# vpecanins/stm32f7-rtlsdr

Hardware: AMD Instinct MI355X
Metric: IQ MSamples/s through FIR+FM-demod+resample (higher is better)
Workload: dtype f32 audio; K2 = u8 x 24-bit fixed-point taps on the i8 matrix pipe, exact i32 sums, one f32 recombination (design Q); K3 / K4 f32; ill-conditioned phases recomputed with the f32 fmaf chain

## Files before the change

### stm32f7-rtlsdr_amd/csrc/sdrfm_q.hip

```cpp
#include <hip/hip_runtime.h>
#include <hip/hip_ext.h>

#include <cstddef>
#include <cstdint>
#include <type_traits>

#include "sdrfm_math.h"
#include "sdrfm_q.h"
#include "sdrfm_b.h"

typedef int qi4_t __attribute__((ext_vector_type(4)));
typedef int qi8_t __attribute__((ext_vector_type(8)));
typedef float qf2_t __attribute__((ext_vector_type(2)));
__device__ void q_raw_buffer_load_lds(qi4_t rsrc, __attribute__((address_space(3))) void* lds, int size, int voffset, int soffset,
                                      int offset, int aux) __asm("llvm.amdgcn.raw.buffer.load.lds");

namespace {

constexpr int QTA = (int)SDRFM_Q_TA;
constexpr int DB0 = 128;
constexpr int ABS = 4;
constexpr int ABW = 128 * ABS;
constexpr int FLW = 64 + 2;
#ifndef SDRFM_Q_GTAB
// ... 39 lines not shown
#define SDRFM_Q_WQB 4
#endif
constexpr int WQB = SDRFM_Q_WQB;
static_assert(WQB >= 4 && WQB <= 16 && 8 * WQB >= (int)SDRFM_Q_TA, "a warm-up holds the d history of a run's first audio output");

__device__ __forceinline__ float q_discriminate(float yr, float yi, float pr, float pi) {
  const float re = __builtin_fmaf(yr, pr, yi * pi);
  const float im = yi * pr - yr * pi;
  const float ax = __builtin_fabsf(re), ay = __builtin_fabsf(im);
  const float mx = __builtin_fmaxf(__builtin_fmaxf(ax, ay), 0x1p-120f), mn = __builtin_fminf(ax, ay);
  const float v = mn * __builtin_amdgcn_rcpf(mx);
  const float s2 = v * v;
  float q = 0x1.e34882p-8f;
  q = __builtin_fmaf(q, s2, -0x1.22fc74p-5f);
  q = __builtin_fmaf(q, s2, 0x1.509024p-4f);
  q = __builtin_fmaf(q, s2, -0x1.12688cp-3f);
  q = __builtin_fmaf(q, s2, 0x1.96c562p-3f);
  q = __builtin_fmaf(q, s2, -0x1.554086p-2f);
  float a = __builtin_fmaf(v, s2 * q, v);
  if (ay > ax) a = 0x1.921fb6p+0f - a;
  if (re < 0.0f) a = 0x1.921fb6p+1f - a;
  return __builtin_copysignf(a, im);
}

__device__ __forceinline__ float q_angle(float yr, float yi, float& mx_out) {
  const float ax = __builtin_fabsf(yr), ay = __builtin_fabsf(yi);
  const float mx = __builtin_fmaxf(__builtin_fmaxf(ax, ay), 0x1p-120f), mn = __builtin_fminf(ax, ay);
  mx_out = mx;
  const float v = mn * __builtin_amdgcn_rcpf(mx);
  const float s2 = v * v;
  float q = 0x1.e34882p-8f;
  q = __builtin_fmaf(q, s2, -0x1.22fc74p-5f);
  q = __builtin_fmaf(q, s2, 0x1.509024p-4f);
  q = __builtin_fmaf(q, s2, -0x1.12688cp-3f);
  q = __builtin_fmaf(q, s2, 0x1.96c562p-3f);
  q = __builtin_fmaf(q, s2, -0x1.554086p-2f);
  float a = __builtin_fmaf(v, s2 * q, v);
  if (ay > ax) a = 0x1.921fb6p+0f - a;
  if (yr < 0.0f) a = 0x1.921fb6p+1f - a;
  return __builtin_copysignf(a, yi);
}
__device__ __forceinline__ float q_wrap(float x) {
  float t = __builtin_fmaf(x, 0x1.45f306p-3f, 0x1.8p+23f);
  asm volatile("" : "+v"(t));
  const float k = t - 0x1.8p+23f;
  return __builtin_fmaf(k, -0x1.921fb6p+2f, x);
}

__device__ __forceinline__ unsigned q_pcm_word(float v) {
  const float c = __builtin_amdgcn_fmed3f(v, -32768.0f, 32767.0f);
  float t = c + 0x1.8p+23f;
  asm volatile("" : "+v"(t));
  return __builtin_amdgcn_perm(__builtin_bit_cast(unsigned, t), __builtin_bit_cast(unsigned, t), 0x05040504u);
}

template <int N>
__device__ __forceinline__ void wait_vmcnt() {
  static_assert(N >= 0 && N < 16, "vmcnt immediate");
  __builtin_amdgcn_s_waitcnt(0x0f70 | N);
}

#ifdef SDRFM_Q_PHASES
#define Q_PHASE(i) do { const unsigned long long tn_ = __builtin_readcyclecounter(); t_ph[i] += tn_ - t_last; t_last = tn_; } while (0)
#else
#define Q_PHASE(i) do { } while (0)
#endif

template <int D, int DA, int NSLOT>
constexpr uint32_t q_lds() { return (uint32_t)(QGeo<D, DA>::PRE + 1024 * NSLOT + 4 * (QGeo<D, DA>::DBW + ABW + FLW + GTW)); }
struct QPcmArgs { SdrfmQParams p; SdrfmSinkChain t; };
static_assert(ABS * 128 <= 64 * (int)SDRFM_CHAIN_CH, "a flush of parked audio is one scan of the wave");
template <int C0, int NSLOT, int D, int DA, bool PCM = false>
__device__ __forceinline__ void mfir_body(const SdrfmQParams& p, const uint32_t bid) {
  using G = QGeo<D, DA>;
  [[maybe_unused]] constexpr int NCH = G::NCH;
  constexpr int QD = D, QDA = DA, NSC = G::NSC, BLKB = G::BLKB, STEPB = G::STEPB, PRE = G::PRE, DBW = G::DBW, RWIN = G::RWIN;
  constexpr bool ALIGNED = G::ALIGNED;
  constexpr int CS = G::CS;
  constexpr int RINGB = NSLOT * 1024;
  static_assert(RINGB % (2 * STEPB) == 0 && (ALIGNED ? NSLOT == 2 * CS : (NSLOT >= 5 && NSLOT - 4 < 16)), "ring: whole pairs of steps");
  extern __shared__ __attribute__((aligned(16))) unsigned char smem[];
  float* const db = reinterpret_cast<float*>(smem + PRE + RINGB);
  float* const ab = db + DBW;
  unsigned short* const fl16 = reinterpret_cast<unsigned short*>(ab + ABW);
  const int lane = (int)threadIdx.x, n = lane & 15, g = lane >> 4;
  const uint32_t si = bid / p.runs, run = bid - si * p.runs;
  const uint32_t stream = p.slist ? p.slist[si] : si;
  const uint32_t Bt = (p.M + 7u) >> 3, Qt = (Bt + WQB - 1u) / WQB, vs = p.iq_prev ? 1u : 0u;
  const uint32_t Gq = Qt + p.runs - 1u + vs;
  const uint32_t e0 = (uint32_t)(((uint64_t)run * Gq) / p.runs), e1 = (uint32_t)(((uint64_t)(run + 1) * Gq) / p.runs);
  const int q0 = run == 0 ? 0 : (int)e0 - (int)(run - 1u + vs), q1 = (int)e1 - (int)(run + vs);
  if (q0 >= q1) return;
  if (lane == 0) *reinterpret_cast<uint2*>(fl16 + 128) = make_uint2(0u, 0u);
#ifdef SDRFM_Q_STAMPS
  unsigned long long* const tsp = p.dbg ? p.dbg + 16 * (size_t)bid : nullptr;
  unsigned long long t_wait = 0, t_first = 0;
  const unsigned long long t_entry = __builtin_amdgcn_s_memrealtime();
  const unsigned long long c_entry = __builtin_readcyclecounter();
#endif
#ifdef SDRFM_Q_PHASES
  unsigned long long t_ph[8] = {0, 0, 0, 0, 0, 0, 0, 0}, t_last = 0;
#endif
  const bool from_prev = run == 0 && p.iq_prev != nullptr;
  const bool warm = run > 0 || from_prev;
  const int b0 = WQB * q0;
  int b1 = WQB * q1;
// ... 207 lines not shown
        q_raw_buffer_load_lds(rsrc, slot_ptr(0), 16, vpos, 0, 0, SDRFM_Q_AUX);
        q_raw_buffer_load_lds(rsrc, slot_ptr(0), 16, vpos, 0, 1024, SDRFM_Q_AUX);
        vpos += 2048;
      }
      return;
    }
    if (k > 0 && !(k & 1)) {
      q_raw_buffer_load_lds(rsrc, slot_ptr(slot), 16, vpos, 0, 0, SDRFM_Q_AUX);
      vpos += 1024;
      slot = (slot + 1 == NSLOT) ? 0 : slot + 1;
    }
    q_raw_buffer_load_lds(rsrc, slot_ptr(slot), 16, vpos, 0, 0, SDRFM_Q_AUX);
    q_raw_buffer_load_lds(rsrc, slot_ptr(slot), 16, vpos, 0, 1024, SDRFM_Q_AUX);
    slot = (slot + 2 >= NSLOT) ? slot + 2 - NSLOT : slot + 2;
    vpos += 2048;
  };
  typedef const __attribute__((address_space(4))) SdrfmQParams* KargPtr;
  auto kargs = [&]() -> KargPtr {
    KargPtr pp = (KargPtr)__builtin_amdgcn_kernarg_segment_ptr();
    asm volatile("" : "+s"(pp));
    return pp;
  };
  int npend = 0, jfl = jg0;
  [[maybe_unused]] float yrun = 0.0f;
  [[maybe_unused]] bool pfirst = true;
  [[maybe_unused]] float* const pstash = reinterpret_cast<float*>(smem + q_lds<D, DA, NSLOT>());
  typedef const __attribute__((address_space(4))) SdrfmSinkChain* KChainPtr;
  [[maybe_unused]] auto kchain = [&]() -> KChainPtr {
    const __attribute__((address_space(4))) unsigned char* pp = (const __attribute__((address_space(4))) unsigned char*)__builtin_amdgcn_kernarg_segment_ptr();
    asm volatile("" : "+s"(pp));
    return (KChainPtr)(pp + offsetof(QPcmArgs, t));
  };
  [[maybe_unused]] unsigned long long pv_early = 0ull;
  [[maybe_unused]] bool published = false;
  [[maybe_unused]] float dp_early = 0.0f;
  auto flush_audio = [&](const bool fin = false) {
    __builtin_amdgcn_wave_barrier();
#if defined(SDRFM_Q_ABLATE) && (SDRFM_Q_ABLATE & 256)
    float* row = p.audio - jfl;
    const int ln_ = lane;
#else
    uint32_t st_ = stream;
    int ln_ = lane;
    asm volatile("" : "+s"(st_), "+v"(ln_));
    float* row = kargs()->audio + (size_t)st_ * kargs()->audio_stride;
#endif
    const int lo = jfl > jlo ? jfl : jlo;
#if defined(SDRFM_Q_ABLATE) && (SDRFM_Q_ABLATE & 128)
    const int hi_ = (ab[lane] == 1234.5f) ? lo + 2 : lo;
#else
    const int hi_ = (j1 < jfl + 128 * npend) ? j1 : jfl + 128 * npend;
#endif
    const int par = (int)((reinterpret_cast<uintptr_t>(row) >> 2) & 1u);
    bool want_audio = true;
    if constexpr (PCM) want_audio = kargs()->audio != nullptr;
    if (want_audio) for (int e = lo - ((lo + par) & 1) + 2 * ln_; e < hi_; e += 128) {
      const bool v0 = e >= lo, v1 = e + 1 < hi_;
      const float a0 = v0 ? ab[e - jfl] : 0.0f, a1 = v1 ? ab[e + 1 - jfl] : 0.0f;
      if constexpr (PCM) {
        if (v0 && v1) __builtin_nontemporal_store(qf2_t{a0, a1}, reinterpret_cast<qf2_t*>(row + e));
        else if (v0) __builtin_nontemporal_store(a0, row + e);
        else if (v1) __builtin_nontemporal_store(a1, row + e + 1);
      } else {
        if (v0 && v1) *reinterpret_cast<qf2_t*>(row + e) = qf2_t{a0, a1};
        else if (v0) row[e] = a0;
        else if (v1) row[e + 1] = a1;
      }
    }
    if constexpr (PCM) {
      const int cntf = hi_ - lo;
      if (cntf > 0) {
        constexpr int PCH = (int)SDRFM_CHAIN_CH, FIX = (int)SDRFM_CHAIN_FIX;
        const KChainPtr tp = kchain();
        const float alpha = tp->alpha, gain = tp->gain;
        asm volatile("s_waitcnt lgkmcnt(0)" ::: "memory");
        __builtin_amdgcn_wave_barrier();
        float* const xa = ab + (lo - jfl);
        unsigned* const xw = reinterpret_cast<unsigned*>(xa);
        const int i0 = PCH * ln_;
        float xr[PCH];
#pragma unroll
        for (int q = 0; q < PCH; ++q) xr[q] = (i0 + q < cntf) ? xa[i0 + q] : 0.0f;
        float sc = 0.0f;
#pragma unroll
        for (int q = 0; q < PCH; ++q) sc = __builtin_fmaf(tp->w[q], xr[q], sc);
        float pw = tp->pc;
        if (ln_ == 0) sc = __builtin_fmaf(pw, yrun, sc);
#pragma unroll
        for (int d = 1; d < 64; d <<= 1) {
          const float o = __shfl_up(sc, (unsigned)d, 64);
          const float sn = __builtin_fmaf(pw, o, sc);
          sc = ln_ >= d ? sn : sc;
          pw *= pw;
        }
        if (fin) {
          const int Ll = (cntf - 1) / PCH, rl = (cntf - 1) % PCH;
          const float ypub = __shfl(sc, Ll, 64) * tp->dinv[PCH - 1 - rl];
          uint32_t bid2 = bid;
          asm volatile("" : "+s"(bid2));
          if (ln_ == 0) {
            const uint32_t call = tp->call, nst = tp->n_streams;
            const unsigned long long w = ((unsigned long long)((last_run ? call : tp->run_call) + 1u) << 32) | __builtin_bit_cast(unsigned, ypub);
            __hip_atomic_store(last_run ? tp->sg + (size_t)((call + 1u) % SDRFM_CHAIN_SG_SLOTS) * nst + st_ : tp->runstate + bid2, w, __ATOMIC_RELAXED,
                               __HIP_MEMORY_SCOPE_AGENT);
            unsigned long long zero = 0ull;
            asm volatile("" : "+v"(zero));
            pv_early = __hip_atomic_fetch_add(run == 0 ? tp->sg + (size_t)(call % SDRFM_CHAIN_SG_SLOTS) * nst + st_ : tp->runstate + (bid2 - 1u), zero,
                                              __ATOMIC_RELAXED, __HIP_MEMORY_SCOPE_AGENT);
          }
          dp_early = ln_ < (int)SDRFM_CHAIN_FIX ? tp->dpow[ln_] : 0.0f;
          published = true;
        }
        float y = __shfl_up(sc, 1u, 64);
        if (ln_ == 0) y = yrun;
        __builtin_amdgcn_wave_barrier();
#pragma unroll
        for (int q = 0; q < PCH; ++q) {
          const float yn = __builtin_fmaf(alpha, xr[q] - y, y);
          y = (i0 + q < cntf) ? yn : y;
          if (i0 + q < cntf) {
            xw[i0 + q] = q_pcm_word(yn * gain);
            if (pfirst && i0 + q < FIX) pstash[i0 + q] = yn;
          }
        }
        yrun = __shfl(y, (cntf - 1) / PCH, 64);
        __builtin_amdgcn_wave_barrier();
        unsigned* const out = reinterpret_cast<unsigned*>(tp->pcm + (size_t)st_ * tp->pcm_stride);
        const int parp = (int)((reinterpret_cast<uintptr_t>(out) >> 2) & 1u), ps = lo + (pfirst ? FIX : 0);
        for (int e = ps - ((ps + parp) & 1) + 2 * ln_; e < hi_; e += 128) {
          const bool v0 = e >= ps, v1 = e + 1 < hi_;
          const unsigned w0 = v0 ? xw[e - lo] : 0u, w1 = v1 ? xw[e + 1 - lo] : 0u;
          if (v0 && v1) *reinterpret_cast<uint2*>(out + e) = make_uint2(w0, w1);
          else if (v0) out[e] = w0;
          else if (v1) out[e + 1] = w1;
        }
        pfirst = false;
      }
    }
    jfl += 128 * npend;
    npend = 0;
  };
  int nflag = 0;
  auto repair_flagged = [&]() {
    int ln = lane;
    uint32_t st = stream;
    asm volatile("" : "+v"(ln), "+s"(st));
    const KargPtr pp = kargs();
#ifdef SDRFM_Q_PHASES
    unsigned long long r_t0 = __builtin_readcyclecounter(), r_t1;
#define R_PHASE(word, shift, waitfirst) do { if (waitfirst) asm volatile("s_waitcnt vmcnt(0) lgkmcnt(0)" ::: "memory"); r_t1 = __builtin_readcyclecounter(); \
                                             t_ph[word] += ((r_t1 - r_t0) & 0xffffffffull) << shift; r_t0 = r_t1; } while (0)
#else
#define R_PHASE(word, shift, waitfirst) do { } while (0)
#endif
    const unsigned char* const row = pp->iq + (size_t)st * pp->iq_stride;
    const unsigned char* const pre = from_prev ? pp->iq_prev + (size_t)st * pp->iq_prev_stride + 2 * (size_t)pp->N_prev
                                               : pp->hist_q_in + (size_t)(2 * QTP) * ((size_t)st + 1);
    unsigned* const cnt = reinterpret_cast<unsigned*>(fl16 + 128);
    __builtin_amdgcn_wave_barrier();
    unsigned nrep = 0;
    for (int e0 = 0; e0 < nflag; e0 += 64) {
      const int e = e0 + ln;
      int l = 0, slot = 0, m0 = (int)pp->M;
      if (e < nflag) {
        const unsigned ent = fl16[e];
        l = (int)(ent & 63u);
        slot = (int)(ent >> 6) - 1;
        m0 = mbase + 128 * slot + 8 * (l & 15) + 2 * (l >> 4);
      }
      const bool act = m0 < (int)pp->M;
      nrep += (unsigned)__builtin_popcountll(__builtin_amdgcn_ballot_w64(act));
      if (act) {
        const int n0 = QD * m0 - QTP;
        uint2 w[RWIN / 4];
#pragma unroll
        for (int c = 0; c < RWIN / 4; ++c) {
          const int n = n0 + 4 * c;
          w[c] = *reinterpret_cast<const uint2*>((n >= 0 ? row : pre) + 2 * (ptrdiff_t)n);
        }
        R_PHASE(0, 0, 0);
        R_PHASE(0, 32, 1);
        qf2_t a[3] = {qf2_t{0.0f, 0.0f}, qf2_t{0.0f, 0.0f}, qf2_t{0.0f, 0.0f}};
        const float* const hz = db;
#pragma unroll
        for (int i = 0; i < RWIN; ++i) {
          const unsigned wd = (i & 2) ? w[i >> 2].y : w[i >> 2].x;
          const qf2_t b = {(float)((wd >> ((i & 1) ? 16 : 0)) & 0xffu), (float)((wd >> ((i & 1) ? 24 : 8)) & 0xffu)};
          const qf2_t x = b - qf2_t{127.5f, 127.5f};
// ... 259 lines not shown
      a0 += a0b;
      a1 += a1b;
      *reinterpret_cast<qf2_t*>(ab + 128 * npend + 2 * lane) = qf2_t{a0, a1};
      ++npend;
      if (osm == QDA) {
        if (lane < QTA) {
          const float hv = db[DB0 + sigma + 128 * QDA - QTA + lane];
          db[DB0 + sigma - QTA + lane] = hv;
        }
        __builtin_amdgcn_wave_barrier();
        osm = 0;
        mbase += 128 * QDA;
      }
      if (npend == ABS) flush_audio();
      Q_PHASE(6);
    }
#if SDRFM_Q_PEEL
  };
  for (int kk = 0; kk < nsteps - 1; ++kk) step(std::false_type{}, kk);
  step(std::true_type{}, nsteps - 1);
#else
  }
#endif
#ifdef SDRFM_Q_STAMPS
  const unsigned long long t_loop = __builtin_amdgcn_s_memrealtime();
#endif
  wait_vmcnt<0>();
  flush_audio(true);
  if constexpr (PCM) {
    const KChainPtr tp = kchain();
    uint32_t st_ = stream, bid_ = bid;
    int ln_ = lane;
    asm volatile("" : "+s"(st_), "+s"(bid_), "+v"(ln_));
    const uint32_t call = tp->call, nst = tp->n_streams;
    unsigned long long* const rs = tp->runstate;
    unsigned long long* const sg = tp->sg;
    const float dp = published ? dp_early : (ln_ < (int)SDRFM_CHAIN_FIX ? tp->dpow[ln_] : 0.0f);
    unsigned long long pv = pv_early;
    if (ln_ == 0) {
      if (!published) {
        const unsigned long long w = ((unsigned long long)((last_run ? call : tp->run_call) + 1u) << 32) | __builtin_bit_cast(unsigned, yrun);
        __hip_atomic_store(last_run ? sg + (size_t)((call + 1u) % SDRFM_CHAIN_SG_SLOTS) * nst + st_ : rs + bid_, w, __ATOMIC_RELAXED, __HIP_MEMORY_SCOPE_AGENT);
      }
      unsigned long long* const src = run == 0 ? sg + (size_t)(call % SDRFM_CHAIN_SG_SLOTS) * nst + st_ : rs + (bid_ - 1u);
      const uint32_t want = run == 0 ? call : tp->run_call + 1u;
      unsigned long long zero = 0ull;
      asm volatile("" : "+v"(zero));
      int it = 0;
      for (;; ++it) {
        if (it > 0 || !published) pv = __hip_atomic_fetch_add(src, zero, __ATOMIC_RELAXED, __HIP_MEMORY_SCOPE_AGENT);
        if ((uint32_t)(pv >> 32) == want || it == (1 << 19)) break;
        __builtin_amdgcn_s_sleep(16);
      }
      if (it == (1 << 19)) { pv = 0ull; __hip_atomic_store(tp->err, 1u, __ATOMIC_RELAXED, __HIP_MEMORY_SCOPE_AGENT); }
    }
    const float carry = __builtin_bit_cast(float, __builtin_amdgcn_readfirstlane((int)(unsigned)pv));
    const int nfix = (j1 - jlo < (int)SDRFM_CHAIN_FIX) ? j1 - jlo : (int)SDRFM_CHAIN_FIX;
    if (ln_ < nfix) {
      const float yv = __builtin_fmaf(dp, carry, pstash[ln_]);
      reinterpret_cast<unsigned*>(tp->pcm + (size_t)st_ * tp->pcm_stride)[jlo + ln_] = q_pcm_word(yv * tp->gain);
    }
  }
  const KargPtr pe = kargs();
  if (pe->n_repaired && lane == 0) {
    const uint2 cnt = *reinterpret_cast<const uint2*>(fl16 + 128);
    if (cnt.y) {
      atomicAdd(pe->n_repaired, cnt.x);
      atomicAdd(pe->n_repaired + 1, cnt.y);
      if (pe->stream_pass) atomicAdd(pe->stream_pass + stream, cnt.y);
    }
  }

  if (last_run && !(SDRFM_Q_HO_RING && !ALIGNED)) {
    const unsigned char* row = pe->iq + (size_t)stream * pe->iq_stride;
    const int HTe = (int)pe->T - 1;
    const size_t Ne = pe->N;
    for (int k = lane; k < HTe; k += 64) {
      const unsigned raw = *reinterpret_cast<const unsigned short*>(row + 2 * (Ne - HTe + k));
      reinterpret_cast<unsigned short*>(pe->hist_b_out)[(size_t)stream * HTe + k] = (unsigned short)raw;
      pe->hist_x_out[(size_t)stream * HTe + k] = make_float2((float)(raw & 0xffu) - 127.5f, (float)(raw >> 8) - 127.5f);
    }
    if (lane < 2 * QTP / 16)
      *reinterpret_cast<qi4_t*>(pe->hist_q_out + (size_t)(2 * QTP) * stream + 16 * lane) =
          *reinterpret_cast<const qi4_t*>(row + 2 * Ne - 2 * QTP + 16 * lane);
  }
#ifdef SDRFM_Q_STAMPS
  if (tsp && lane == 0) {
    tsp[0] = t_entry; tsp[1] = t_first; tsp[2] = t_loop; tsp[3] = __builtin_amdgcn_s_memrealtime(); tsp[4] = t_wait;
#ifdef SDRFM_Q_PHASES
    for (int i = 0; i < 8; ++i) tsp[8 + i] = t_ph[i];
#endif
    tsp[5] = (__builtin_amdgcn_s_getreg((3 << 11) | 20) & 7) | ((unsigned long long)__builtin_amdgcn_s_getreg((31 << 11) | 4) << 8);
    tsp[6] = (unsigned long long)nsteps; tsp[7] = __builtin_readcyclecounter() - c_entry;
  }
#endif
}


template <int C0, int NSLOT, int D, int DA>
__global__ void __launch_bounds__(64) __attribute__((amdgpu_waves_per_eu(D == 16 ? 3 : 4))) k_mfir(SdrfmQParams p) {
  mfir_body<C0, NSLOT, D, DA>(p, blockIdx.x);
}

template <int C0, int NSLOT, int D, int DA>
__global__ void __launch_bounds__(64) __attribute__((amdgpu_waves_per_eu(D == 16 ? 3 : 4))) k_mfir_pcm(QPcmArgs a) {
  mfir_body<C0, NSLOT, D, DA, true>(a.p, blockIdx.x);
}
// ... 207 lines not shown
```

### stm32f7-rtlsdr_amd/csrc/sdrfm_sink.hip

```cpp
#include <hip/hip_runtime.h>
#include <hip/hip_ext.h>

#include <cmath>
#include <cstdint>
#include <cstdio>
#include <cstring>
#include <new>

#include "../../include/sdrfm.h"
#include "sdrfm_sink_chain.h"

namespace {

struct SinkParams {
  const float* audio;
  size_t audio_stride;
  int16_t* pcm;
  size_t pcm_stride;
  const unsigned long long* sg_in;
  unsigned long long* sg_out;
  uint32_t gen_next;
  uint32_t n_streams, n;
  float alpha, gain;
};
// ... 2 lines not shown
  __shared__ unsigned tile[64 * 65];
  const uint32_t lane = threadIdx.x;
  const uint32_t s0 = blockIdx.x * 64;
  const uint32_t rows = (p.n_streams - s0 < 64u) ? p.n_streams - s0 : 64u;
  const uint32_t mine = s0 + lane;
  float y = (lane < rows) ? __uint_as_float((unsigned)p.sg_in[mine]) : 0.0f;
  for (uint32_t t0 = 0; t0 < p.n; t0 += 64) {
    const uint32_t cols = (p.n - t0 < 64u) ? p.n - t0 : 64u;
    if (lane < cols)
      for (uint32_t r = 0; r < rows; ++r)
        tile[r * 65 + lane] = __float_as_uint(p.audio[(size_t)(s0 + r) * p.audio_stride + t0 + lane]);
    __syncthreads();
    if (lane < rows) {
      for (uint32_t i = 0; i < cols; ++i) {
        const float x = __uint_as_float(tile[lane * 65 + i]);
        y = __builtin_fmaf(p.alpha, x - y, y);
        float v = y * p.gain;
        if (v > 32767.0f) v = 32767.0f;
        if (v < -32768.0f) v = -32768.0f;
        const unsigned s = (unsigned)(int)__builtin_rintf(v) & 0xffffu;
        tile[lane * 65 + i] = s | (s << 16);
      }
    }
    __syncthreads();
    if (lane < cols)
      for (uint32_t r = 0; r < rows; ++r)
        reinterpret_cast<unsigned*>(p.pcm + (size_t)(s0 + r) * p.pcm_stride)[t0 + lane] = tile[r * 65 + lane];
    __syncthreads();
  }
  if (lane < rows) p.sg_out[mine] = ((unsigned long long)p.gen_next << 32) | __float_as_uint(y);
}

constexpr uint32_t SINK_NT = 256, SINK_C = 19, SINK_SEG = SINK_NT * SINK_C;
static_assert(SINK_NT == 256, "four waves: the carries between them are combined by hand");
template <bool LIST>
__global__ void __launch_bounds__(256) k_pcm_sink_scan(SinkParams p, float pc, const uint32_t* list, uint32_t* err) {
  __shared__ float x[SINK_SEG];
  __shared__ float sc[4];
  unsigned* const xw = reinterpret_cast<unsigned*>(x);
  const uint32_t s = LIST ? list[blockIdx.x] : blockIdx.x, t = threadIdx.x;
  const float* const row = p.audio + (size_t)s * p.audio_stride;
  unsigned* const out = reinterpret_cast<unsigned*>(p.pcm + (size_t)s * p.pcm_stride);
  float y0;
  if constexpr (LIST) {
    if (t == 0) {
      unsigned long long pv = 0ull, zero = 0ull;
      asm volatile("" : "+v"(zero));
      int it = 0;
      for (;; ++it) {
        pv = __hip_atomic_fetch_add(const_cast<unsigned long long*>(p.sg_in) + s, zero, __ATOMIC_RELAXED, __HIP_MEMORY_SCOPE_AGENT);
        if ((uint32_t)(pv >> 32) == p.gen_next - 1u || it == (1 << 19)) break;
        __builtin_amdgcn_s_sleep(16);
      }
      if (it == (1 << 19)) { pv = 0ull; __hip_atomic_store(err, 1u, __ATOMIC_RELAXED, __HIP_MEMORY_SCOPE_AGENT); }
      sc[0] = __uint_as_float((unsigned)pv);
    }
    __syncthreads();
    y0 = sc[0];
    __syncthreads();
  } else {
    y0 = __uint_as_float((unsigned)p.sg_in[s]);
  }
  for (uint32_t base = 0; base < p.n; base += SINK_SEG) {
    const uint32_t m = (p.n - base < SINK_SEG) ? p.n - base : SINK_SEG;
#pragma unroll
    for (uint32_t q = 0; q < SINK_C; ++q) {
      const uint32_t i = t + SINK_NT * q;
      if (i < m) x[i] = row[base + i];
    }
    __syncthreads();
    const uint32_t i0 = t * SINK_C < m ? t * SINK_C : m, cnt = (m - i0 < SINK_C) ? m - i0 : SINK_C;
    float xr[SINK_C];
#pragma unroll
    for (uint32_t q = 0; q < SINK_C; ++q) xr[q] = q < cnt ? x[i0 + q] : 0.0f;
    float y = t == 0 ? y0 : 0.0f;
#pragma unroll
    for (uint32_t q = 0; q < SINK_C; ++q)
      if (q < cnt) y = __builtin_fmaf(p.alpha, xr[q] - y, y);
    const uint32_t wl = t & 63u, wv = t >> 6;
    float sv = y, pw = pc;
#pragma unroll
    for (uint32_t d = 1; d < 64u; d <<= 1) {
      const float o = __shfl_up(sv, d, 64);
      const float sn = __builtin_fmaf(pw, o, sv);
      sv = wl >= d ? sn : sv;
      pw *= pw;
    }
    if (wl == 63u) sc[wv] = sv;
    float pl = 1.0f, pb = pc;
#pragma unroll
    for (uint32_t bit = 0; bit < 6u; ++bit) {
      pl = ((wl >> bit) & 1u) ? pl * pb : pl;
      pb *= pb;
    }
    const float prev = __shfl_up(sv, 1u, 64);
    __syncthreads();
    float cw = 0.0f;
    if (wv >= 1u) cw = sc[0];
    if (wv >= 2u) cw = __builtin_fmaf(pw, cw, sc[1]);
    if (wv >= 3u) cw = __builtin_fmaf(pw, cw, sc[2]);
    y = wl == 0u ? (wv == 0u ? y0 : cw) : __builtin_fmaf(pl, cw, prev);
    __syncthreads();
#pragma unroll
    for (uint32_t q = 0; q < SINK_C; ++q)
      if (q < cnt) {
        y = __builtin_fmaf(p.alpha, xr[q] - y, y);
        float v = y * p.gain;
        if (v > 32767.0f) v = 32767.0f;
        if (v < -32768.0f) v = -32768.0f;
        const unsigned w = (unsigned)(int)__builtin_rintf(v) & 0xffffu;
        xw[i0 + q] = w | (w << 16);
      }
    if (cnt > 0 && i0 + cnt == m) sc[0] = y;
    __syncthreads();
    y0 = sc[0];
#pragma unroll
    for (uint32_t q = 0; q < SINK_C; ++q) {
      const uint32_t i = t + SINK_NT * q;
      if (i < m) out[base + i] = xw[i];
    }
    __syncthreads();
  }
  if (t == 0) {
    const unsigned long long w = ((unsigned long long)p.gen_next << 32) | __float_as_uint(y0);
    if constexpr (LIST) __hip_atomic_store(p.sg_out + s, w, __ATOMIC_RELAXED, __HIP_MEMORY_SCOPE_AGENT);
    else p.sg_out[s] = w;
  }
}

}

struct sdrfm_pcm_sink {
  uint32_t n_streams;
  float alpha, gain;
  int device;
  hipStream_t own_stream, stream;
  unsigned long long* d_sg;
  float* d_dpow;
  uint32_t calls;
  float* d_audio;
  int16_t* d_pcm;
  uint32_t cap;
};

#define STRY(expr, code)                                                                                       \
  do {                                                                                                         \
    hipError_t e__ = (expr);                                                                                   \
    if (e__ != hipSuccess) {                                                                                   \
      fprintf(stderr, "[sdrfm] %s failed: %s (%s:%d)\n", #expr, hipGetErrorString(e__), __FILE__, __LINE__);  \
      return (code);                                                                                           \
    }                                                                                                          \
  } while (0)

static void sink_free(sdrfm_pcm_sink* k) {
  if (!k) return;
  (void)hipSetDevice(k->device);
  if (k->d_sg) (void)hipFree(k->d_sg);
  if (k->d_dpow) (void)hipFree(k->d_dpow);
  if (k->d_audio) (void)hipFree(k->d_audio);
  if (k->d_pcm) (void)hipFree(k->d_pcm);
  if (k->own_stream) (void)hipStreamDestroy(k->own_stream);
  delete k;
}

int sdrfm_sink_chain_params(sdrfm_pcm_sink* k, int device, uint32_t n_streams, SdrfmSinkChain* out) {
  if (!k || !out || k->device != device || k->n_streams != n_streams) return 0;
  out->pcm = nullptr; out->pcm_stride = 0; out->runstate = nullptr; out->run_call = 0;
  out->sg = k->d_sg; out->n_streams = n_streams; out->dpow = k->d_dpow; out->err = reinterpret_cast<uint32_t*>(k->d_dpow + SDRFM_CHAIN_FIX);
  out->call = k->calls;
  out->alpha = k->alpha; out->gain = k->gain;
  out->pc = (float)pow(1.0 - (double)k->alpha, (double)SDRFM_CHAIN_CH);
  for (uint32_t q = 0; q < SDRFM_CHAIN_CH; ++q) out->w[q] = (float)((double)k->alpha * pow(1.0 - (double)k->alpha, (double)(SDRFM_CHAIN_CH - 1u - q)));
  for (uint32_t q = 0; q < SDRFM_CHAIN_CH; ++q) out->dinv[q] = (float)pow(1.0 - (double)k->alpha, -(double)q);
  return k->alpha >= SDRFM_CHAIN_MIN_ALPHA ? 2 : 1;
}

void sdrfm_sink_chain_issued(sdrfm_pcm_sink* k) { ++k->calls; }

int sdrfm_sink_launch_on(sdrfm_pcm_sink* k, const float* audio, size_t audio_stride, uint32_t n, int16_t* pcm, size_t pcm_stride, hipStream_t stream) {
  if (!k) return SDRFM_EINVAL;
  if (n == 0) return SDRFM_OK;
  SinkParams p;
  p.sg_in = k->d_sg + (size_t)(k->calls % SDRFM_CHAIN_SG_SLOTS) * k->n_streams; p.sg_out = k->d_sg + (size_t)((k->calls + 1u) % SDRFM_CHAIN_SG_SLOTS) * k->n_streams;
  p.n_streams = k->n_streams; p.n = n; p.alpha = k->alpha; p.gain = k->gain;
  p.gen_next = k->calls + 1u;
  p.audio = audio; p.audio_stride = audio_stride; p.pcm = pcm; p.pcm_stride = pcm_stride;
  hipLaunchKernelGGL(k_pcm_sink_scan<false>, dim3(k->n_streams), dim3(SINK_NT), 0, stream, p, (float)pow(1.0 - (double)k->alpha, (double)SINK_C), nullptr, nullptr);
  STRY(hipGetLastError(), SDRFM_FAIL);
  ++k->calls;
  return SDRFM_OK;
}

int sdrfm_sink_launch_list_on(sdrfm_pcm_sink* k, const SdrfmSinkChain& c, const uint32_t* list_dev, uint32_t n_list, const float* audio, size_t audio_stride, uint32_t n,
                              int16_t* pcm, size_t pcm_stride, hipStream_t stream, hipEvent_t done) {
  if (!k || !list_dev) return SDRFM_EINVAL;
  if (n == 0 || n_list == 0) return SDRFM_OK;
  SinkParams p;
  p.sg_in = k->d_sg + (size_t)(c.call % SDRFM_CHAIN_SG_SLOTS) * k->n_streams; p.sg_out = k->d_sg + (size_t)((c.call + 1u) % SDRFM_CHAIN_SG_SLOTS) * k->n_streams;
  p.n_streams = k->n_streams; p.n = n; p.alpha = k->alpha; p.gain = k->gain;
  p.gen_next = c.call + 1u;
  p.audio = audio; p.audio_stride = audio_stride; p.pcm = pcm; p.pcm_stride = pcm_stride;
  hipExtLaunchKernelGGL(k_pcm_sink_scan<true>, dim3(n_list), dim3(SINK_NT), 0, stream, nullptr, done, 0, p, (float)pow(1.0 - (double)k->alpha, (double)SINK_C), list_dev, c.err);
  STRY(hipGetLastError(), SDRFM_FAIL);
  return SDRFM_OK;
}

extern "C" {

int sdrfm_pcm_sink_create(uint32_t n_streams, float alpha, float gain, int32_t device, sdrfm_pcm_sink_t** out) {
  if (!out) return SDRFM_EINVAL;
  *out = nullptr;
  if (!n_streams || !(alpha > 0.0f) || alpha > 1.0f || !(gain == gain)) return SDRFM_EINVAL;
  int ndev = 0;
  if (hipGetDeviceCount(&ndev) != hipSuccess || ndev <= 0 || device < 0 || device >= ndev) return SDRFM_NO_DEVICE;
  hipDeviceProp_t prop;
  if (hipGetDeviceProperties(&prop, device) != hipSuccess || strncmp(prop.gcnArchName, "gfx950", 6) != 0) return SDRFM_NO_DEVICE;
  STRY(hipSetDevice(device), SDRFM_NO_DEVICE);
  sdrfm_pcm_sink* k = new (std::nothrow) sdrfm_pcm_sink();
  if (!k) return SDRFM_ENOMEM;
  memset(static_cast<void*>(k), 0, sizeof(*k));
  k->n_streams = n_streams; k->alpha = alpha; k->gain = gain; k->device = device;
  if (hipStreamCreateWithFlags(&k->own_stream, hipStreamNonBlocking) != hipSuccess ||
      hipMalloc(&k->d_sg, sizeof(unsigned long long) * SDRFM_CHAIN_SG_SLOTS * n_streams) != hipSuccess ||
      hipMalloc(&k->d_dpow, sizeof(float) * (SDRFM_CHAIN_FIX + 1)) != hipSuccess) { sink_free(k); return SDRFM_ENOMEM; }
  {
    float dp[SDRFM_CHAIN_FIX + 1];
    for (uint32_t i = 0; i < SDRFM_CHAIN_FIX; ++i) dp[i] = (float)pow(1.0 - (double)alpha, (double)(i + 1));
    dp[SDRFM_CHAIN_FIX] = 0.0f;
    if (hipMemcpy(k->d_dpow, dp, sizeof(dp), hipMemcpyHostToDevice) != hipSuccess) { sink_free(k); return SDRFM_FAIL; }
  }
  k->stream = k->own_stream;
  const int rc = sdrfm_pcm_sink_reset(k);
  if (rc != SDRFM_OK) { sink_free(k); return rc; }
  *out = k;
  return SDRFM_OK;
}

void sdrfm_pcm_sink_destroy(sdrfm_pcm_sink_t* k) {
  if (!k) return;
  (void)hipSetDevice(k->device);
  (void)hipStreamSynchronize(k->stream);
  sink_free(k);
}

int sdrfm_pcm_sink_reset(sdrfm_pcm_sink_t* k) {
  if (!k) return SDRFM_EINVAL;
  STRY(hipSetDevice(k->device), SDRFM_FAIL);
  STRY(hipMemsetAsync(k->d_sg, 0, sizeof(unsigned long long) * SDRFM_CHAIN_SG_SLOTS * k->n_streams, k->stream), SDRFM_FAIL);
  STRY(hipMemsetAsync(k->d_dpow + SDRFM_CHAIN_FIX, 0, sizeof(uint32_t), k->stream), SDRFM_FAIL);
  STRY(hipStreamSynchronize(k->stream), SDRFM_FAIL);
  k->calls = 0;
  return SDRFM_OK;
}

int sdrfm_pcm_sink_set_stream(sdrfm_pcm_sink_t* k, void* hip_stream) {
  if (!k) return SDRFM_EINVAL;
  STRY(hipSetDevice(k->device), SDRFM_FAIL);
  STRY(hipStreamSynchronize(k->stream), SDRFM_FAIL);
  k->stream = hip_stream ? static_cast<hipStream_t>(hip_stream) : k->own_stream;
  return SDRFM_OK;
}

static int sink_chain_error(sdrfm_pcm_sink* k) {
  uint32_t e = 0;
  if (hipMemcpy(&e, k->d_dpow + SDRFM_CHAIN_FIX, sizeof(e), hipMemcpyDeviceToHost) != hipSuccess) return SDRFM_FAIL;
  if (e) fprintf(stderr, "[sdrfm] PCM sink: a run of a demodulator launch waited in vain for its predecessor's state (csrc/sdrfm_sink_chain.h)\n");
  return e ? SDRFM_FAIL : SDRFM_OK;
}

int sdrfm_pcm_sink_synchronize(sdrfm_pcm_sink_t* k) {
  if (!k) return SDRFM_EINVAL;
  STRY(hipSetDevice(k->device), SDRFM_FAIL);
  STRY(hipStreamSynchronize(k->stream), SDRFM_FAIL);
  return sink_chain_error(k);
}

int sdrfm_pcm_sink_process_batch(sdrfm_pcm_sink_t* k, const float* audio, size_t audio_stride, uint32_t n, int16_t* pcm,
                                 size_t pcm_stride, uint32_t flags) {
  if (!k) return SDRFM_EINVAL;
  if (flags & ~(SDRFM_F_DEVICE_PTRS | SDRFM_PCM_F_EXACT)) return SDRFM_EINVAL;
  if (n == 0) return SDRFM_OK;
  if (!audio || !pcm) return SDRFM_EINVAL;
  if (k->n_streams > 1 && (audio_stride < n || pcm_stride < 2 * (size_t)n)) return SDRFM_ECAPACITY;
  if (pcm_stride & 1u) return SDRFM_EINVAL;
  STRY(hipSetDevice(k->device), SDRFM_FAIL);
  SinkParams p;
  p.sg_in = k->d_sg + (size_t)(k->calls % SDRFM_CHAIN_SG_SLOTS) * k->n_streams; p.sg_out = k->d_sg + (size_t)((k->calls + 1u) % SDRFM_CHAIN_SG_SLOTS) * k->n_streams;
  p.n_streams = k->n_streams; p.n = n; p.alpha = k->alpha; p.gain = k->gain;
  p.gen_next = k->calls + 1u;
  const dim3 grid((k->n_streams + 63) / 64);
  const float pc = (float)pow(1.0 - (double)k->alpha, (double)SINK_C);
  const bool exact = (flags & SDRFM_PCM_F_EXACT) != 0;
  auto launch = [&]() {
    if (exact) hipLaunchKernelGGL(k_pcm_sink, grid, dim3(64), 0, k->stream, p);
    else hipLaunchKernelGGL(k_pcm_sink_scan<false>, dim3(k->n_streams), dim3(SINK_NT), 0, k->stream, p, pc, nullptr, nullptr);
  };
  if (flags & SDRFM_F_DEVICE_PTRS) {
    if ((uintptr_t)pcm % 4 != 0) return SDRFM_EINVAL;
    p.audio = audio; p.audio_stride = audio_stride; p.pcm = pcm; p.pcm_stride = pcm_stride;
    launch();
    STRY(hipGetLastError(), SDRFM_FAIL);
    ++k->calls;
    return SDRFM_OK;
  }
  if (n > k->cap) {
    if (k->d_audio) (void)hipFree(k->d_audio);
    if (k->d_pcm) (void)hipFree(k->d_pcm);
    k->d_audio = nullptr; k->d_pcm = nullptr; k->cap = 0;
    const uint32_t cap = (n + 1023u) & ~1023u;
    if (hipMalloc(&k->d_audio, sizeof(float) * (size_t)cap * k->n_streams) != hipSuccess ||
        hipMalloc(&k->d_pcm, sizeof(int16_t) * 2 * (size_t)cap * k->n_streams) != hipSuccess) return SDRFM_ENOMEM;
    k->cap = cap;
  }
  const size_t as = (k->n_streams > 1) ? audio_stride : n, ps = (k->n_streams > 1) ? pcm_stride : 2 * (size_t)n;
  STRY(hipMemcpy2DAsync(k->d_audio, sizeof(float) * k->cap, audio, sizeof(float) * as, sizeof(float) * n, k->n_streams,
                        hipMemcpyHostToDevice, k->stream), SDRFM_FAIL);
  p.audio = k->d_audio; p.audio_stride = k->cap; p.pcm = k->d_pcm; p.pcm_stride = 2 * (size_t)k->cap;
  launch();
// ... 22 lines not shown
```

Before: 2.631 million.

## Fuse final PCM flush into register path with DPP scan and mapped error flag

On the final flush of the PCM path, audio is now stored straight from registers using aligned 4-wide chunk stores, and the output is no longer written back to LDS first. The cross-lane prefix scan moves from __shfl_up to permlane/DPP moves, and the broadcasts use readlane. The sink's error flag moves from device memory to mapped, coherent host memory, so checking it needs only a host read instead of a blocking hipMemcpy. The cost is extra code complexity, system-scope atomics when a wait times out, and reliance on gfx950 permlane swap intrinsics.

Result: no change. 2.622 million, median of 3 (-0.4%).

```diff
diff --git a/stm32f7-rtlsdr_amd/csrc/sdrfm_q.hip b/stm32f7-rtlsdr_amd/csrc/sdrfm_q.hip
--- a/stm32f7-rtlsdr_amd/csrc/sdrfm_q.hip
+++ b/stm32f7-rtlsdr_amd/csrc/sdrfm_q.hip
@@ -115,6 +115,77 @@
   float t = c + 0x1.8p+23f;
   asm volatile("" : "+v"(t));
   return __builtin_amdgcn_perm(__builtin_bit_cast(unsigned, t), __builtin_bit_cast(unsigned, t), 0x05040504u);
+}
+
+__device__ __forceinline__ float q_row_up(float v, int lane) {
+  const unsigned u = __builtin_bit_cast(unsigned, v);
+  const auto a = __builtin_amdgcn_permlane16_swap(u, u, false, false);
+  const auto b = __builtin_amdgcn_permlane32_swap(a[1], a[1], false, false);
+  return __builtin_bit_cast(float, (lane >> 4) == 2 ? b[0] : a[0]);
+}
+template <int DIST>
+__device__ __forceinline__ float q_lanes_up(float v, int lane) {
+  static_assert(DIST == 1 || DIST == 2 || DIST == 4 || DIST == 8 || DIST == 16 || DIST == 32, "a scan step");
+  if constexpr (DIST == 32) {
+    const unsigned u = __builtin_bit_cast(unsigned, v);
+    return __builtin_bit_cast(float, __builtin_amdgcn_permlane32_swap(u, u, false, false)[0]);
+  } else if constexpr (DIST == 16) {
+    return q_row_up(v, lane);
+  } else if constexpr (DIST == 1) {
+    return __builtin_bit_cast(float, __builtin_amdgcn_update_dpp(__builtin_bit_cast(int, v), __builtin_bit_cast(int, v), 0x138, 0xF, 0xF, false));
+  } else {
+    const float up = q_row_up(v, lane);
+    const float z = (lane & 15) >= 16 - DIST ? up : v;
+    return __builtin_bit_cast(float, __builtin_amdgcn_update_dpp(0, __builtin_bit_cast(int, z), 0x120 + DIST, 0xF, 0xF, false));
+  }
+}
+typedef unsigned qu2_t __attribute__((ext_vector_type(2)));
+typedef unsigned qu4_t __attribute__((ext_vector_type(4)));
+typedef qu2_t qu2a_t __attribute__((aligned(4)));
+typedef qu4_t qu4a_t __attribute__((aligned(4)));
+template <bool NT, int OFF, int N, class W>
+__device__ __forceinline__ void q_store_piece(unsigned* base, W& word, int e, int a, int b) {
+  static_assert((N == 1 || N == 2 || N == 4) && OFF + N <= 8, "a piece of a lane's chunk");
+  unsigned v[N];
+#pragma unroll
+  for (int i = 0; i < N; ++i) v[i] = word(OFF + i);
+  const int f = e + OFF;
+  if (N > 1 && f >= a && f + N <= b) {
+    if constexpr (N == 4) {
+      const qu4_t x = {v[0], v[1], v[2], v[3]};
+      if constexpr (NT) __builtin_nontemporal_store(x, reinterpret_cast<qu4a_t*>(base + f));
+      else *reinterpret_cast<qu4a_t*>(base + f) = x;
+    } else if constexpr (N == 2) {
+      const qu2_t x = {v[0], v[1]};
+      if constexpr (NT) __builtin_nontemporal_store(x, reinterpret_cast<qu2a_t*>(base + f));
+      else *reinterpret_cast<qu2a_t*>(base + f) = x;
+    }
+  } else if (f < b && f + N > a) {
+#pragma unroll
+    for (int i = 0; i < N; ++i)
+      if (f + i >= a && f + i < b) {
+        if constexpr (NT) __builtin_nontemporal_store(v[i], base + f + i);
+        else base[f + i] = v[i];
+      }
+  }
+}
+#ifndef SDRFM_Q_TAIL_UNALIGNED
+#define SDRFM_Q_TAIL_UNALIGNED 0
+#endif
+template <bool NT, class W>
+__device__ __forceinline__ void q_store_chunk(unsigned* base, W word, int elo, int e, int a, int b) {
+  const int k = SDRFM_Q_TAIL_UNALIGNED ? 0 : (int)((reinterpret_cast<uintptr_t>(base + elo) >> 2) & 3u);
+  if (k == 0) {
+    q_store_piece<NT, 0, 4>(base, word, e, a, b); q_store_piece<NT, 4, 4>(base, word, e, a, b);
+  } else if (k == 2) {
+    q_store_piece<NT, 0, 2>(base, word, e, a, b); q_store_piece<NT, 2, 4>(base, word, e, a, b); q_store_piece<NT, 6, 2>(base, word, e, a, b);
+  } else if (k == 1) {
+    q_store_piece<NT, 0, 1>(base, word, e, a, b); q_store_piece<NT, 1, 2>(base, word, e, a, b); q_store_piece<NT, 3, 4>(base, word, e, a, b);
+    q_store_piece<NT, 7, 1>(base, word, e, a, b);
+  } else {
+    q_store_piece<NT, 0, 1>(base, word, e, a, b); q_store_piece<NT, 1, 4>(base, word, e, a, b); q_store_piece<NT, 5, 2>(base, word, e, a, b);
+    q_store_piece<NT, 7, 1>(base, word, e, a, b);
+  }
 }
 
 template <int N>
@@ -428,50 +499,113 @@
     const int hi_ = (j1 < jfl + 128 * npend) ? j1 : jfl + 128 * npend;
 #endif
     const int par = (int)((reinterpret_cast<uintptr_t>(row) >> 2) & 1u);
-    bool want_audio = true;
-    if constexpr (PCM) want_audio = kargs()->audio != nullptr;
-    if (want_audio) for (int e = lo - ((lo + par) & 1) + 2 * ln_; e < hi_; e += 128) {
-      const bool v0 = e >= lo, v1 = e + 1 < hi_;
-      const float a0 = v0 ? ab[e - jfl] : 0.0f, a1 = v1 ? ab[e + 1 - jfl] : 0.0f;
+    if (!PCM || !fin) {
+      bool want_audio = true;
+      if constexpr (PCM) want_audio = kargs()->audio != nullptr;
+      if (want_audio) for (int e = lo - ((lo + par) & 1) + 2 * ln_; e < hi_; e += 128) {
+        const bool v0 = e >= lo, v1 = e + 1 < hi_;
+        const float a0 = v0 ? ab[e - jfl] : 0.0f, a1 = v1 ? ab[e + 1 - jfl] : 0.0f;
+        if constexpr (PCM) {
+          if (v0 && v1) __builtin_nontemporal_store(qf2_t{a0, a1}, reinterpret_cast<qf2_t*>(row + e));
+          else if (v0) __builtin_nontemporal_store(a0, row + e);
+          else if (v1) __builtin_nontemporal_store(a1, row + e + 1);
+        } else {
+          if (v0 && v1) *reinterpret_cast<qf2_t*>(row + e) = qf2_t{a0, a1};
+          else if (v0) row[e] = a0;
+          else if (v1) row[e + 1] = a1;
+        }
+      }
       if constexpr (PCM) {
-        if (v0 && v1) __builtin_nontemporal_store(qf2_t{a0, a1}, reinterpret_cast<qf2_t*>(row + e));
-        else if (v0) __builtin_nontemporal_store(a0, row + e);
-        else if (v1) __builtin_nontemporal_store(a1, row + e + 1);
-      } else {
-        if (v0 && v1) *reinterpret_cast<qf2_t*>(row + e) = qf2_t{a0, a1};
-        else if (v0) row[e] = a0;
-        else if (v1) row[e + 1] = a1;
-      }
-    }
-    if constexpr (PCM) {
+        const int cntf = hi_ - lo;
+        if (cntf > 0) {
+          constexpr int PCH = (int)SDRFM_CHAIN_CH, FIX = (int)SDRFM_CHAIN_FIX;
+          const KChainPtr tp = kchain();
+          const float alpha = tp->alpha, gain = tp->gain;
+          asm volatile("s_waitcnt lgkmcnt(0)" ::: "memory");
+          __builtin_amdgcn_wave_barrier();
+          float* const xa = ab + (lo - jfl);
+          unsigned* const xw = reinterpret_cast<unsigned*>(xa);
+          const int i0 = PCH * ln_;
+          float xr[PCH];
+#pragma unroll
+          for (int q = 0; q < PCH; ++q) xr[q] = (i0 + q < cntf) ? xa[i0 + q] : 0.0f;
+          float sc = 0.0f;
+#pragma unroll
+          for (int q = 0; q < PCH; ++q) sc = __builtin_fmaf(tp->w[q], xr[q], sc);
+          float pw = tp->pc;
+          if (ln_ == 0) sc = __builtin_fmaf(pw, yrun, sc);
+#pragma unroll
+          for (int d = 1; d < 64; d <<= 1) {
+            const float o = __shfl_up(sc, (unsigned)d, 64);
+            const float sn = __builtin_fmaf(pw, o, sc);
+            sc = ln_ >= d ? sn : sc;
+            pw *= pw;
+          }
+          float y = __shfl_up(sc, 1u, 64);
+          if (ln_ == 0) y = yrun;
+          __builtin_amdgcn_wave_barrier();
+#pragma unroll
+          for (int q = 0; q < PCH; ++q) {
+            const float yn = __builtin_fmaf(alpha, xr[q] - y, y);
+            y = (i0 + q < cntf) ? yn : y;
+            if (i0 + q < cntf) {
+              xw[i0 + q] = q_pcm_word(yn * gain);
+              if (pfirst && i0 + q < FIX) pstash[i0 + q] = yn;
+            }
+          }
+          yrun = __shfl(y, (cntf - 1) / PCH, 64);
+          __builtin_amdgcn_wave_barrier();
+          unsigned* const out = reinterpret_cast<unsigned*>(tp->pcm + (size_t)st_ * tp->pcm_stride);
+          const int parp = (int)((reinterpret_cast<uintptr_t>(out) >> 2) & 1u), ps = lo + (pfirst ? FIX : 0);
+          for (int e = ps - ((ps + parp) & 1) + 2 * ln_; e < hi_; e += 128) {
+            const bool v0 = e >= ps, v1 = e + 1 < hi_;
+            const unsigned w0 = v0 ? xw[e - lo] : 0u, w1 = v1 ? xw[e + 1 - lo] : 0u;
+            if (v0 && v1) *reinterpret_cast<uint2*>(out + e) = make_uint2(w0, w1);
+            else if (v0) out[e] = w0;
+            else if (v1) out[e + 1] = w1;
+          }
+          pfirst = false;
+        }
+      }
+    } else if constexpr (PCM) {
       const int cntf = hi_ - lo;
       if (cntf > 0) {
         constexpr int PCH = (int)SDRFM_CHAIN_CH, FIX = (int)SDRFM_CHAIN_FIX;
         const KChainPtr tp = kchain();
         const float alpha = tp->alpha, gain = tp->gain;
-        asm volatile("s_waitcnt lgkmcnt(0)" ::: "memory");
-        __builtin_amdgcn_wave_barrier();
-        float* const xa = ab + (lo - jfl);
-        unsigned* const xw = reinterpret_cast<unsigned*>(xa);
+        float pw = tp->pc, wq_[PCH];
+#pragma unroll
+        for (int q = 0; q < PCH; ++q) wq_[q] = tp->w[q];
+        const bool want_audio = kargs()->audio != nullptr;
+        const float* const xa = ab + (lo - jfl);
         const int i0 = PCH * ln_;
         float xr[PCH];
 #pragma unroll
         for (int q = 0; q < PCH; ++q) xr[q] = (i0 + q < cntf) ? xa[i0 + q] : 0.0f;
+        if (want_audio) {
+          auto aword = [&](int q) { return __builtin_bit_cast(unsigned, xr[q]); };
+          q_store_chunk<true>(reinterpret_cast<unsigned*>(row), aword, lo, lo + i0, lo, hi_);
+        }
         float sc = 0.0f;
 #pragma unroll
-        for (int q = 0; q < PCH; ++q) sc = __builtin_fmaf(tp->w[q], xr[q], sc);
-        float pw = tp->pc;
+        for (int q = 0; q < PCH; ++q) sc = __builtin_fmaf(wq_[q], xr[q], sc);
         if (ln_ == 0) sc = __builtin_fmaf(pw, yrun, sc);
-#pragma unroll
-        for (int d = 1; d < 64; d <<= 1) {
-          const float o = __shfl_up(sc, (unsigned)d, 64);
+        auto scan_step = [&](auto dist) {
+          constexpr int d = decltype(dist)::value;
+          const float o = q_lanes_up<d>(sc, ln_);
           const float sn = __builtin_fmaf(pw, o, sc);
           sc = ln_ >= d ? sn : sc;
           pw *= pw;
-        }
-        if (fin) {
+        };
+        scan_step(std::integral_constant<int, 1>{});
+        scan_step(std::integral_constant<int, 2>{});
+        scan_step(std::integral_constant<int, 4>{});
+        scan_step(std::integral_constant<int, 8>{});
+        scan_step(std::integral_constant<int, 16>{});
+        scan_step(std::integral_constant<int, 32>{});
+        {
           const int Ll = (cntf - 1) / PCH, rl = (cntf - 1) % PCH;
-          const float ypub = __shfl(sc, Ll, 64) * tp->dinv[PCH - 1 - rl];
+          const float ypub = __builtin_bit_cast(float, __builtin_amdgcn_readlane(__builtin_bit_cast(int, sc), Ll)) * tp->dinv[PCH - 1 - rl];
           uint32_t bid2 = bid;
           asm volatile("" : "+s"(bid2));
           if (ln_ == 0) {
@@ -487,29 +621,18 @@
           dp_early = ln_ < (int)SDRFM_CHAIN_FIX ? tp->dpow[ln_] : 0.0f;
           published = true;
         }
-        float y = __shfl_up(sc, 1u, 64);
+        float y = q_lanes_up<1>(sc, ln_);
         if (ln_ == 0) y = yrun;
-        __builtin_amdgcn_wave_barrier();
-#pragma unroll
-        for (int q = 0; q < PCH; ++q) {
+        auto walk = [&](int q) {
           const float yn = __builtin_fmaf(alpha, xr[q] - y, y);
           y = (i0 + q < cntf) ? yn : y;
-          if (i0 + q < cntf) {
-            xw[i0 + q] = q_pcm_word(yn * gain);
-            if (pfirst && i0 + q < FIX) pstash[i0 + q] = yn;
-          }
-        }
-        yrun = __shfl(y, (cntf - 1) / PCH, 64);
+          if (pfirst && i0 + q < cntf && i0 + q < FIX) pstash[i0 + q] = yn;
+          return q_pcm_word(yn * gain);
+        };
+        unsigned* const out = reinterpret_cast<unsigned*>(tp->pcm + (size_t)st_ * tp->pcm_stride);
+        q_store_chunk<false>(out, walk, lo, lo + i0, lo + (pfirst ? FIX : 0), hi_);
+        yrun = __builtin_bit_cast(float, __builtin_amdgcn_readlane(__builtin_bit_cast(int, y), (cntf - 1) / PCH));
         __builtin_amdgcn_wave_barrier();
-        unsigned* const out = reinterpret_cast<unsigned*>(tp->pcm + (size_t)st_ * tp->pcm_stride);
-        const int parp = (int)((reinterpret_cast<uintptr_t>(out) >> 2) & 1u), ps = lo + (pfirst ? FIX : 0);
-        for (int e = ps - ((ps + parp) & 1) + 2 * ln_; e < hi_; e += 128) {
-          const bool v0 = e >= ps, v1 = e + 1 < hi_;
-          const unsigned w0 = v0 ? xw[e - lo] : 0u, w1 = v1 ? xw[e + 1 - lo] : 0u;
-          if (v0 && v1) *reinterpret_cast<uint2*>(out + e) = make_uint2(w0, w1);
-          else if (v0) out[e] = w0;
-          else if (v1) out[e + 1] = w1;
-        }
         pfirst = false;
       }
     }
@@ -875,7 +998,7 @@
         if ((uint32_t)(pv >> 32) == want || it == (1 << 19)) break;
         __builtin_amdgcn_s_sleep(16);
       }
-      if (it == (1 << 19)) { pv = 0ull; __hip_atomic_store(tp->err, 1u, __ATOMIC_RELAXED, __HIP_MEMORY_SCOPE_AGENT); }
+      if (it == (1 << 19)) { pv = 0ull; __hip_atomic_store(tp->err, 1u, __ATOMIC_RELAXED, __HIP_MEMORY_SCOPE_SYSTEM); }
     }
     const float carry = __builtin_bit_cast(float, __builtin_amdgcn_readfirstlane((int)(unsigned)pv));
     const int nfix = (j1 - jlo < (int)SDRFM_CHAIN_FIX) ? j1 - jlo : (int)SDRFM_CHAIN_FIX;
diff --git a/stm32f7-rtlsdr_amd/csrc/sdrfm_sink.hip b/stm32f7-rtlsdr_amd/csrc/sdrfm_sink.hip
--- a/stm32f7-rtlsdr_amd/csrc/sdrfm_sink.hip
+++ b/stm32f7-rtlsdr_amd/csrc/sdrfm_sink.hip
@@ -78,7 +78,7 @@
         if ((uint32_t)(pv >> 32) == p.gen_next - 1u || it == (1 << 19)) break;
         __builtin_amdgcn_s_sleep(16);
       }
-      if (it == (1 << 19)) { pv = 0ull; __hip_atomic_store(err, 1u, __ATOMIC_RELAXED, __HIP_MEMORY_SCOPE_AGENT); }
+      if (it == (1 << 19)) { pv = 0ull; __hip_atomic_store(err, 1u, __ATOMIC_RELAXED, __HIP_MEMORY_SCOPE_SYSTEM); }
       sc[0] = __uint_as_float((unsigned)pv);
     }
     __syncthreads();
@@ -163,6 +163,8 @@
   hipStream_t own_stream, stream;
   unsigned long long* d_sg;
   float* d_dpow;
+  uint32_t* h_err;
+  uint32_t* d_err;
   uint32_t calls;
   float* d_audio;
   int16_t* d_pcm;
@@ -183,6 +185,7 @@
   (void)hipSetDevice(k->device);
   if (k->d_sg) (void)hipFree(k->d_sg);
   if (k->d_dpow) (void)hipFree(k->d_dpow);
+  if (k->h_err) (void)hipHostFree(k->h_err);
   if (k->d_audio) (void)hipFree(k->d_audio);
   if (k->d_pcm) (void)hipFree(k->d_pcm);
   if (k->own_stream) (void)hipStreamDestroy(k->own_stream);
@@ -192,7 +195,7 @@
 int sdrfm_sink_chain_params(sdrfm_pcm_sink* k, int device, uint32_t n_streams, SdrfmSinkChain* out) {
   if (!k || !out || k->device != device || k->n_streams != n_streams) return 0;
   out->pcm = nullptr; out->pcm_stride = 0; out->runstate = nullptr; out->run_call = 0;
-  out->sg = k->d_sg; out->n_streams = n_streams; out->dpow = k->d_dpow; out->err = reinterpret_cast<uint32_t*>(k->d_dpow + SDRFM_CHAIN_FIX);
+  out->sg = k->d_sg; out->n_streams = n_streams; out->dpow = k->d_dpow; out->err = k->d_err;
   out->call = k->calls;
   out->alpha = k->alpha; out->gain = k->gain;
   out->pc = (float)pow(1.0 - (double)k->alpha, (double)SDRFM_CHAIN_CH);
@@ -248,11 +251,12 @@
   k->n_streams = n_streams; k->alpha = alpha; k->gain = gain; k->device = device;
   if (hipStreamCreateWithFlags(&k->own_stream, hipStreamNonBlocking) != hipSuccess ||
       hipMalloc(&k->d_sg, sizeof(unsigned long long) * SDRFM_CHAIN_SG_SLOTS * n_streams) != hipSuccess ||
-      hipMalloc(&k->d_dpow, sizeof(float) * (SDRFM_CHAIN_FIX + 1)) != hipSuccess) { sink_free(k); return SDRFM_ENOMEM; }
+      hipMalloc(&k->d_dpow, sizeof(float) * SDRFM_CHAIN_FIX) != hipSuccess ||
+      hipHostMalloc(reinterpret_cast<void**>(&k->h_err), sizeof(uint32_t), hipHostMallocMapped | hipHostMallocCoherent) != hipSuccess) { sink_free(k); return SDRFM_ENOMEM; }
+  if (hipHostGetDevicePointer(reinterpret_cast<void**>(&k->d_err), k->h_err, 0) != hipSuccess) { sink_free(k); return SDRFM_FAIL; }
   {
-    float dp[SDRFM_CHAIN_FIX + 1];
+    float dp[SDRFM_CHAIN_FIX];
     for (uint32_t i = 0; i < SDRFM_CHAIN_FIX; ++i) dp[i] = (float)pow(1.0 - (double)alpha, (double)(i + 1));
-    dp[SDRFM_CHAIN_FIX] = 0.0f;
     if (hipMemcpy(k->d_dpow, dp, sizeof(dp), hipMemcpyHostToDevice) != hipSuccess) { sink_free(k); return SDRFM_FAIL; }
   }
   k->stream = k->own_stream;
@@ -273,8 +277,8 @@
   if (!k) return SDRFM_EINVAL;
   STRY(hipSetDevice(k->device), SDRFM_FAIL);
   STRY(hipMemsetAsync(k->d_sg, 0, sizeof(unsigned long long) * SDRFM_CHAIN_SG_SLOTS * k->n_streams, k->stream), SDRFM_FAIL);
-  STRY(hipMemsetAsync(k->d_dpow + SDRFM_CHAIN_FIX, 0, sizeof(uint32_t), k->stream), SDRFM_FAIL);
-  STRY(hipStreamSynchronize(k->stream), SDRFM_FAIL);
+  STRY(hipStreamSynchronize(k->stream), SDRFM_FAIL);
+  *static_cast<volatile uint32_t*>(k->h_err) = 0u;
   k->calls = 0;
   return SDRFM_OK;
 }
@@ -288,8 +292,7 @@
 }
 
 static int sink_chain_error(sdrfm_pcm_sink* k) {
-  uint32_t e = 0;
-  if (hipMemcpy(&e, k->d_dpow + SDRFM_CHAIN_FIX, sizeof(e), hipMemcpyDeviceToHost) != hipSuccess) return SDRFM_FAIL;
+  const uint32_t e = *static_cast<volatile uint32_t*>(k->h_err);
   if (e) fprintf(stderr, "[sdrfm] PCM sink: a run of a demodulator launch waited in vain for its predecessor's state (csrc/sdrfm_sink_chain.h)\n");
   return e ? SDRFM_FAIL : SDRFM_OK;
 }
```
